# Ham3798/shielded-pool-pinocchio-solana

Measured on AMD Instinct MI355X. Metric: Groth16 proofs/sec, higher is better.
Workload: dtype u32x8 (254-bit Montgomery integers); 1 GPU; audit_circuit (RLWE, const-PK; scripts/generate_audit.py:246-465), batch of 2048 independent proofs per GPU per step, every row a distinct witness; circuit=audit, n_constraints=29178, n_wires=35432, domain=32768, batch_per_gpu=2048, n_distinct_witnesses=2048, table_bytes=226725433344, parallelism=independent proofs x1, pk_bytes=9850060

## Files before the change

### shielded-pool-pinocchio-solana_amd/csrc/bn254.hpp

```cpp
#pragma once
#include <stdint.h>
#include <stddef.h>
#include "bn254_consts.hpp"

#if defined(__HIPCC__)
#include <hip/hip_runtime.h>
#define SPP_HD __host__ __device__ __forceinline__
#define SPP_UNROLL _Pragma("unroll")
#else
#define SPP_HD inline
#define SPP_UNROLL
#endif

namespace spp {

SPP_HD uint32_t addc32(uint32_t a, uint32_t b, uint32_t& carry) {
#if defined(__clang__)
  unsigned co;
  uint32_t r = __builtin_addc(a, b, carry, &co);
  carry = co;
  return r;
#else
  uint64_t t = (uint64_t)a + b + carry;
  carry = (uint32_t)(t >> 32);
// ... 175 lines not shown
    to9(l, a9);
    SPP_UNROLL for (int i = 0; i < 9; i++) d9[i] = a9[i] << 1;
    uint64_t c[18];
    SPP_UNROLL for (int k = 0; k < 18; k++) c[k] = 0;
    SPP_UNROLL for (int i = 0; i < 9; i++) {
      c[2 * i] += (uint64_t)a9[i] * a9[i];
      SPP_UNROLL for (int j = i + 1; j < 9; j++) c[i + j] += (uint64_t)a9[i] * d9[j];
    }
    return reduce_columns(c);
  }

  SPP_HD Fp mul_small(uint32_t k) const {
    Fp acc = zero();
    Fp base = *this;
    while (k) {
      if (k & 1) acc = acc + base;
      base = base.dbl();
      k >>= 1;
    }
    return acc;
  }

  SPP_HD void to_canonical(uint32_t out[8]) const {
    Fp o;
    SPP_UNROLL for (int i = 0; i < 8; i++) o.l[i] = (i == 0);
    Fp c = *this * o;
    cond_sub(c.l);
    SPP_UNROLL for (int i = 0; i < 8; i++) out[i] = c.l[i];
  }
  static SPP_HD Fp from_canonical(const uint32_t in[8]) {
    Fp a;
    SPP_UNROLL for (int i = 0; i < 8; i++) a.l[i] = in[i];
    return a * r2();
  }
  static SPP_HD Fp from_u256(const uint32_t in[8]) {
    Fp a;
    SPP_UNROLL for (int i = 0; i < 8; i++) a.l[i] = in[i];
    for (int k = 0; k < 6; k++) cond_sub(a.l);
    return a * r2();
  }
  static SPP_HD Fp from_u64(uint64_t v) {
    uint32_t c[8];
    SPP_UNROLL for (int i = 0; i < 8; i++) c[i] = 0;
    c[0] = (uint32_t)v;
    c[1] = (uint32_t)(v >> 32);
    return from_canonical(c);
  }
  SPP_HD void to_bytes_be(uint8_t out[32]) const {
    uint32_t c[8];
// ... 339 lines not shown
```

### shielded-pool-pinocchio-solana_amd/csrc/kernels.hpp

```cpp
#pragma once
#include <hip/hip_runtime.h>
#include <stdint.h>
#include "bn254.hpp"
#include "f29.hpp"
#include "msm_plan.hpp"
#include "msm_ragged.hpp"
#include "rlwe_ntt.hpp"

namespace spp {

struct DevSparse {
  const uint32_t* rowptr;
  const uint32_t* wire;
  const uint32_t* coeff;
  const uint32_t* lit;
};
static constexpr uint32_t COEFF_ONE = 0x80000000u;
static constexpr uint32_t COEFF_MINUS_ONE = 0x40000000u;
static constexpr uint32_t COEFF_MASK = 0x3fffffffu;

struct HashConsts {
  const Fr* pos3_rc;  const Fr* pos3_mds;
  const Fr* pos5_rc;  const Fr* pos5_mds;
  const Fr* p2_rc;    const Fr* p2_mu;
  const uint32_t* pos3_mds29;
  const uint32_t* pos5_mds29;
};

struct DevCircuit {
  DevSparse A, B, C, H;
  const Fr* coeffs;
  const Fr* aux;
  const uint32_t* program;
  uint32_t n_wires, n_constraints, n_public, n_inputs, challenge_wire;
  const uint32_t* run_start;
  uint32_t n_runs;
  uint32_t max_row_terms;
  const uint8_t* row_flags;
  const uint32_t* sm_wires;
  const int32_t* sm_lo;
  uint32_t sm_nslots;
  const uint32_t* sm_rowptr;
  const uint32_t* sm_slot;
  const int32_t* sm_coef;
  const uint32_t* sm_rest_ptr;
  const uint32_t* sm_rest_wire;
  const uint32_t* sm_rest_coeff;
  const uint32_t* sm_row_out;
  uint32_t sm_nrows;
  const uint8_t* row_small;
  const uint32_t* lg_rows;
  uint32_t lg_n;
  const uint8_t* row_long;
  HashConsts hc;
// ... 112 lines not shown
void launch_scale_rows(hipStream_t st, Fr* data, const Fr* table, uint32_t n, uint32_t P, uint32_t nbatch, size_t batch_stride);
void launch_qap_pointwise(hipStream_t st, Fr* abc, uint32_t n, uint32_t P, Fr zinv);
void launch_qap_product(hipStream_t st, Fr* abc, uint32_t n, uint32_t P);

template <class F>
struct MsmWalk;
template <>
struct MsmWalk<Fq> {
  static constexpr uint32_t waves_per_simd = 3;
  static constexpr uint32_t rows_waves_per_simd = 2;
  static constexpr int product_form = F29_SCAN;
  static constexpr uint32_t occ(uint32_t Wt) { return Wt == 1 ? waves_per_simd : rows_waves_per_simd; }
};
template <>
struct MsmWalk<Fq2> {
  static constexpr uint32_t waves_per_simd = 2;
  static constexpr uint32_t rows_waves_per_simd = 1;
  static constexpr int product_form = F29_COLUMNS;
  static constexpr uint32_t occ(uint32_t Wt) { return Wt == 1 ? waves_per_simd : rows_waves_per_simd; }
};
template <class F>
void launch_build_table(hipStream_t st, const Affine<F>* bases, uint32_t N, uint32_t c, uint32_t Wt, uint32_t row0, uint32_t nrows,
                        Affine<F>* table, XYZZ<F>* tmp, F* tmp_pre, const MsmBlock* blocks = nullptr, uint32_t E = 0);
void launch_msm_digits(hipStream_t st, const uint32_t* rows, const Fr* scalars, int16_t* dig, uint32_t N, uint32_t P, uint32_t c);
template <class F>
void launch_msm_accumulate(hipStream_t st, const Affine<F>* table, const MsmBlock* blocks, const int16_t* dig, XYZZ<F>* partial, uint32_t N, uint32_t P,
                           uint32_t c, const MsmPlan& pl, hipEvent_t ev_start = nullptr, hipEvent_t ev_stop = nullptr, uint32_t* redo_count = nullptr);
template <class F>
void launch_msm_reduce(hipStream_t st, XYZZ<F>* partial, XYZZ<F>* out, uint32_t P, const MsmPlan& pl, uint32_t c, bool empty);
static constexpr uint32_t MSM_FOLD_SETS = 8;
static constexpr uint32_t MSM_FOLD_RADIX = 8;
template <class F>
struct MsmFoldSets {
  XYZZ<F>* partial[MSM_FOLD_SETS];
  XYZZ<F>* out[MSM_FOLD_SETS];
  uint32_t Sg[MSM_FOLD_SETS], R[MSM_FOLD_SETS], c[MSM_FOLD_SETS];
  uint32_t cur[MSM_FOLD_SETS], half[MSM_FOLD_SETS];
};
template <class F>
void launch_msm_reduce_multi(hipStream_t st, MsmFoldSets<F> fs, uint32_t nsets, uint32_t P);

void launch_g1_eval_basis(hipStream_t st, const G1Affine* pts, uint32_t n_pts, uint32_t logn, const Fr* scale, const Fr* tw_inv, G1XYZZ* work,
                          G1Affine* out);

void launch_g1_column_sums(hipStream_t st, const G1Affine* base, const uint32_t* row, const Fr* coeff, uint32_t nterms, const uint32_t* seg,
                           uint32_t nseg, G1XYZZ* work, G1Affine* out);

// ... 31 lines not shown
```

### shielded-pool-pinocchio-solana_amd/csrc/kernels_msm.hip

```cpp
#include "msm_table.hpp"

namespace spp {

template void launch_build_table<Fq>(hipStream_t, const Affine<Fq>*, uint32_t, uint32_t, uint32_t, uint32_t, uint32_t, Affine<Fq>*,
                                     XYZZ<Fq>*, Fq*, const MsmBlock*, uint32_t);
template void launch_msm_accumulate<Fq>(hipStream_t, const Affine<Fq>*, const MsmBlock*, const int16_t*, XYZZ<Fq>*, uint32_t, uint32_t, uint32_t,
                                        const MsmPlan&, hipEvent_t, hipEvent_t, uint32_t*);
template void launch_msm_reduce_multi<Fq>(hipStream_t, MsmFoldSets<Fq>, uint32_t, uint32_t);
template void launch_msm_reduce<Fq>(hipStream_t, XYZZ<Fq>*, XYZZ<Fq>*, uint32_t, const MsmPlan&, uint32_t, bool);
template void launch_fixed_base_mul<Fq>(hipStream_t, const Affine<Fq>*, uint32_t, const Fr*, uint32_t, Affine<Fq>*);

__global__ void __launch_bounds__(256) k_msm_digits(const uint32_t* __restrict__ rows, const Fr* __restrict__ scalars,
                                                    int16_t* __restrict__ dig, uint32_t N, uint32_t P, uint32_t Pp, uint32_t c, uint32_t W) {
  const uint64_t g = (uint64_t)blockIdx.x * blockDim.x + threadIdx.x;
  const uint32_t p = (uint32_t)(g % Pp), i = (uint32_t)(g / Pp);
  if (i >= N || p >= P) return;
  const Fr s = scalars[(size_t)rows[i] * P + p];
  uint32_t l[8];
  s.to_canonical(l);
  const bool neg = canonical_gt_half<FrParams>(l);
  if (neg) {
    uint32_t t[8];
    canonical_negate<FrParams>(l, t);
    SPP_UNROLL for (int k = 0; k < 8; k++) l[k] = t[k];
  }
  const uint32_t mask = (1u << c) - 1u, half = 1u << (c - 1);
  uint32_t carry = 0;
  int16_t* out = dig + (size_t)i * Pp + p;
  const size_t plane = (size_t)N * Pp;
#pragma unroll 1
  for (uint32_t j = 0; j < W; j++) {
    const uint32_t d = (l[0] & mask) + carry;
    SPP_UNROLL for (int k = 0; k < 7; k++) l[k] = (l[k] >> c) | (l[k + 1] << (32 - c));
    l[7] >>= c;
    const bool over = neg ? d > half : d >= half;
    int v = over ? (int)d - (int)(1u << c) : (int)d;
    carry = over ? 1u : 0u;
    if (neg) v = -v;
    out[(size_t)j * plane] = (int16_t)v;
  }
}
void launch_msm_digits(hipStream_t st, const uint32_t* rows, const Fr* scalars, int16_t* dig, uint32_t N, uint32_t P, uint32_t c) {
  if (N == 0 || P == 0) return;
  const uint32_t Pp = msm_padded_batch(P);
  const uint64_t lanes = (uint64_t)N * Pp;
  hipLaunchKernelGGL(k_msm_digits, dim3((uint32_t)((lanes + 255) / 256)), dim3(256), 0, st, rows, scalars, dig, N, P, Pp, c, msm_windows(c));
}

__device__ __forceinline__ XYZZ<Fq> g1_scalar_mul(const XYZZ<Fq>& pt, const Fr& k) {
  uint32_t c[8];
  k.to_canonical(c);
  XYZZ<Fq> acc = XYZZ<Fq>::infinity();
  if (pt.is_inf()) return acc;
#pragma unroll 1
  for (int w = 7; w >= 0; w--) {
    const uint32_t word = w == 0 ? c[0] : w == 1 ? c[1] : w == 2 ? c[2] : w == 3 ? c[3] : w == 4 ? c[4] : w == 5 ? c[5] : w == 6 ? c[6] : c[7];
#pragma unroll 1
    for (int bit = 31; bit >= 0; bit--) {
      acc.dbl_inplace();
      if ((word >> bit) & 1) acc.add(pt);
    }
  }
  return acc;
}
__global__ void __launch_bounds__(64) k_g1_dft_load(const G1Affine* __restrict__ pts, uint32_t n_pts, const Fr* __restrict__ scale,
                                                    G1XYZZ* __restrict__ x, uint32_t n) {
  const uint32_t j = blockIdx.x * blockDim.x + threadIdx.x;
  if (j >= n) return;
  x[j] = j < n_pts ? g1_scalar_mul(G1XYZZ::from_affine(pts[j]), scale[j]) : G1XYZZ::infinity();
// ... 51 lines not shown
```

### shielded-pool-pinocchio-solana_amd/csrc/kernels_solve.hip

```cpp
#include "kernels.hpp"
#include "circuit.hpp"
#include "poseidon29.hpp"
#include "poseidon2.hpp"
#include "gnark_hints.hpp"
#include "sha256.hpp"

namespace spp {

__device__ __forceinline__ Fr dev_row_dot(const DevSparse& m, const Fr* __restrict__ coeffs, uint32_t k, uint32_t k_end_skip,
                                           const Fr* __restrict__ W, uint32_t P, uint32_t p, uint32_t first = 0, uint32_t step = 1) {
  Fr acc = Fr::zero();
  const uint32_t b = m.rowptr[k] + first, e = m.rowptr[k + 1] - k_end_skip;
  for (uint32_t t = b; t < e; t += step) {
    const uint32_t ci = m.coeff[t];
    Fr w = W[(size_t)m.wire[t] * P + p];
    if (ci & COEFF_ONE) acc = acc + w;
    else if (ci & COEFF_MINUS_ONE) acc = acc - w;
    else acc = acc + coeffs[ci & COEFF_MASK] * w;
  }
  return acc;
}

__global__ void __launch_bounds__(256) k_load_inputs(const uint8_t* __restrict__ in_be, const uint8_t* __restrict__ rs_be,
                                                     Fr* __restrict__ W, uint32_t n_inputs, uint32_t n_wires, uint32_t P) {
// ... 699 lines not shown
  if (lanes) hipLaunchKernelGGL(k_count8_hist, dim3((uint32_t)((lanes + 255) / 256)), dim3(256), 0, st, dc, W, counters, h0, n, P);
  hipLaunchKernelGGL(k_count8_store, dim3((256 * P + 255) / 256), dim3(256), 0, st, counters, W, out0, P);
}

__device__ __forceinline__ void wide_mac(uint32_t (&acc)[10], uint32_t c, const Fr& x) {
  uint32_t carry = 0;
  SPP_UNROLL for (int i = 0; i < 8; i++) {
    const uint64_t t = (uint64_t)c * x.l[i] + acc[i] + carry;
    acc[i] = (uint32_t)t;
    carry = (uint32_t)(t >> 32);
  }
  const uint64_t t = (uint64_t)acc[8] + carry;
  acc[8] = (uint32_t)t;
  acc[9] += (uint32_t)(t >> 32);
}
__device__ __forceinline__ Fr wide_finish(const uint32_t (&acc)[10]) {
  Fr lo;
  SPP_UNROLL for (int i = 0; i < 8; i++) lo.l[i] = acc[i];
  Fr::cond_sub_2p(lo.l);
  Fr::cond_sub_2p(lo.l);
  if ((acc[8] | acc[9]) == 0) return lo;
  return lo + Fr::from_u64((uint64_t)acc[8] | ((uint64_t)acc[9] << 32));
}
__device__ __forceinline__ Fr dev_row_dot_wide(const DevSparse& m, const Fr* __restrict__ coeffs, uint32_t k, const Fr* __restrict__ W,
                                                uint32_t P, uint32_t p, uint32_t first = 0, uint32_t step = 1) {
  Fr acc = Fr::zero();
  uint32_t pos[10], neg[10];
  SPP_UNROLL for (int i = 0; i < 10; i++) pos[i] = neg[i] = 0;
  bool any = false;
  const uint32_t b = m.rowptr[k] + first, e = m.rowptr[k + 1];
  for (uint32_t t = b; t < e; t += step) {
    const uint32_t ci = m.coeff[t], li = m.lit[t];
    const Fr w = W[(size_t)m.wire[t] * P + p];
    if (ci & COEFF_ONE) acc = acc + w;
    else if (ci & COEFF_MINUS_ONE) acc = acc - w;
    else if (li) {
      any = true;
      if (li & 0x80000000u) wide_mac(neg, li & 0x7fffffffu, w);
      else wide_mac(pos, li, w);
    } else acc = acc + coeffs[ci & COEFF_MASK] * w;
  }
  if (any) acc = acc + wide_finish(pos) - wide_finish(neg);
  return acc;
}

__global__ void __launch_bounds__(256) k_small_extract(DevCircuit dc, const Fr* __restrict__ W, int16_t* __restrict__ small, uint32_t P,
                                                       uint32_t* __restrict__ status) {
  const uint64_t g = (uint64_t)blockIdx.x * blockDim.x + threadIdx.x;
  if (g >= (uint64_t)dc.sm_nslots * P) return;
  const uint32_t p = (uint32_t)(g % P), s = (uint32_t)(g / P);
  uint32_t c[8], n[8];
  W[(size_t)dc.sm_wires[s] * P + p].to_canonical(c);
  canonical_negate<FrParams>(c, n);
  const bool pos = (c[1] | c[2] | c[3] | c[4] | c[5] | c[6] | c[7]) == 0 && c[0] < 32768u;
  const bool neg = (n[1] | n[2] | n[3] | n[4] | n[5] | n[6] | n[7]) == 0 && n[0] <= 32768u && (c[0] | c[1] | c[2] | c[3] | c[4] | c[5] | c[6] | c[7]) != 0;
  int v = pos ? (int)c[0] : neg ? -(int)n[0] : 0;
  const int lo = dc.sm_lo[s];
  if ((!pos && !neg) || v < lo || v > lo + 255) {
    atomicOr(&status[p], 1u);
    v = 0;
  }
  small[g] = (int16_t)v;
}
__global__ void __launch_bounds__(256) k_spmv_small_rows(DevCircuit dc, const int16_t* __restrict__ small, const Fr* __restrict__ W,
// ... 7 lines not shown
  const uint32_t ro = dc.sm_row_out[r], mat = ro >> 30, k = ro & 0x3fffffffu;
  const Fr mag = Fr::from_u64((uint64_t)(acc < 0 ? -acc : acc));
  Fr v = acc < 0 ? mag.neg() : mag;
  for (uint32_t t = dc.sm_rest_ptr[r]; t < dc.sm_rest_ptr[r + 1]; t++) v = v + dc.coeffs[dc.sm_rest_coeff[t]] * W[(size_t)dc.sm_rest_wire[t] * P + p];
  abc[(size_t)mat * n * P + (size_t)k * P + p] = v;
}

__global__ void __launch_bounds__(256) k_spmv_check(DevCircuit dc, const Fr* __restrict__ W, Fr* __restrict__ abc, uint32_t n, uint32_t P,
                                                    uint32_t* __restrict__ status) {
  const uint64_t g = (uint64_t)blockIdx.x * blockDim.x + threadIdx.x;
  const uint64_t lanes = (uint64_t)(dc.n_runs + (n - dc.n_constraints)) * P;
  if (g >= lanes) return;
  const uint32_t p = (uint32_t)(g % P), r = (uint32_t)(g / P);
  const uint64_t total = (uint64_t)n * P;
  if (r >= dc.n_runs) {
    const uint64_t o = (uint64_t)(dc.n_constraints + (r - dc.n_runs)) * P + p;
    abc[o] = Fr::zero();
    abc[total + o] = Fr::zero();
    abc[2 * total + o] = Fr::zero();
    return;
  }
  const uint32_t k0 = dc.run_start[r], k1 = dc.run_start[r + 1];
  const uint8_t* __restrict__ rs = dc.row_small;
  const Fr b = (rs && (rs[k0] & 2)) ? abc[total + (uint64_t)k0 * P + p] : dev_row_dot_wide(dc.B, dc.coeffs, k0, W, P, p);
  bool bad = false;
  for (uint32_t k = k0; k < k1; k++) {
    const uint64_t o = (uint64_t)k * P + p;
    const uint32_t f = rs ? rs[k] : 0u;
    const Fr a = (f & 1) ? abc[o] : dev_row_dot_wide(dc.A, dc.coeffs, k, W, P, p);
    const Fr c = (f & 4) ? abc[2 * total + o] : dev_row_dot_wide(dc.C, dc.coeffs, k, W, P, p);
    bad |= (a * b != c);
    abc[o] = a;
    abc[total + o] = b;
    abc[2 * total + o] = c;
  }
  if (bad) atomicOr(&status[p], 1u);
}
static constexpr uint32_t LONG_G = 16;
__global__ void __launch_bounds__(1024) k_spmv_long_rows(DevCircuit dc, const Fr* __restrict__ W, Fr* __restrict__ abc, uint32_t n, uint32_t P) {
  __shared__ Fr part[LONG_G][64];
  const uint32_t lane = threadIdx.x & 63, sub = threadIdx.x >> 6, p = blockIdx.x * 64 + lane;
  const uint32_t code = dc.lg_rows[blockIdx.y], mi = code >> 30, k = code & 0x3fffffffu;
  const DevSparse& m = mi == 0 ? dc.A : mi == 1 ? dc.B : dc.C;
  part[sub][lane] = p < P ? dev_row_dot_wide(m, dc.coeffs, k, W, P, p, sub, LONG_G) : Fr::zero();
  __syncthreads();
  if (sub != 0 || p >= P) return;
  Fr acc = part[0][lane];
  SPP_UNROLL for (uint32_t q = 1; q < LONG_G; q++) acc = acc + part[q][lane];
  abc[(uint64_t)mi * n * P + (uint64_t)k * P + p] = acc;
}

static constexpr uint32_t SPMV_G = 16;
__device__ __forceinline__ Fr group_sum(Fr v) {
  SPP_UNROLL for (uint32_t off = SPMV_G / 2; off >= 1; off >>= 1) {
    Fr o;
    SPP_UNROLL for (int i = 0; i < 8; i++) o.l[i] = __shfl_xor(v.l[i], off);
    v = v + o;
  }
  return v;
}
__global__ void __launch_bounds__(256) k_spmv_check_rows(DevCircuit dc, const Fr* __restrict__ W, Fr* __restrict__ abc, uint32_t n, uint32_t P,
                                                         uint32_t* __restrict__ status) {
  const uint64_t g = (uint64_t)blockIdx.x * blockDim.x + threadIdx.x;
  const uint64_t total = (uint64_t)n * P;
  const uint64_t e = g / SPMV_G;
  const uint32_t sub = (uint32_t)(g % SPMV_G);
  const bool live = e < total;
  const uint32_t p = live ? (uint32_t)(e % P) : 0, k = live ? (uint32_t)(e / P) : dc.n_constraints;
  Fr a = Fr::zero(), b = Fr::zero(), c = Fr::zero();
  if (k < dc.n_constraints) {
    a = dev_row_dot_wide(dc.A, dc.coeffs, k, W, P, p, sub, SPMV_G);
    b = dev_row_dot_wide(dc.B, dc.coeffs, k, W, P, p, sub, SPMV_G);
    c = dev_row_dot_wide(dc.C, dc.coeffs, k, W, P, p, sub, SPMV_G);
  }
  a = group_sum(a);
  b = group_sum(b);
  c = group_sum(c);
  if (!live || sub != 0) return;
  if (a * b != c) atomicOr(&status[p], 1u);
  abc[e] = a;
  abc[total + e] = b;
  abc[2 * total + e] = c;
}
void launch_spmv_check(hipStream_t st, DevCircuit dc, const Fr* W, Fr* abc, uint32_t n, uint32_t P, uint32_t* status, int16_t* small) {
  if ((uint64_t)dc.n_runs * P < 65536 || (P <= 64 && dc.max_row_terms > 1024)) {
    const uint64_t lanes = (uint64_t)n * P * SPMV_G;
    hipLaunchKernelGGL(k_spmv_check_rows, dim3((uint32_t)((lanes + 255) / 256)), dim3(256), 0, st, dc, W, abc, n, P, status);
    return;
  }
  if (small && dc.sm_nrows) {
    const uint64_t l1 = (uint64_t)dc.sm_nslots * P, l2 = (uint64_t)dc.sm_nrows * P;
    hipLaunchKernelGGL(k_small_extract, dim3((uint32_t)((l1 + 255) / 256)), dim3(256), 0, st, dc, W, small, P, status);
    hipLaunchKernelGGL(k_spmv_small_rows, dim3((uint32_t)((l2 + 255) / 256)), dim3(256), 0, st, dc, small, W, abc, n, P);
  } else {
    dc.row_small = dc.row_long;
  }
// ... 7 lines not shown
```

### shielded-pool-pinocchio-solana_amd/csrc/msm_table.hpp

```cpp
#pragma once
#include <hip/hip_ext.h>
#include "kernels.hpp"
#include <algorithm>
#include "f29.hpp"

namespace spp {

static constexpr unsigned MSM_FOLD_COOP_MAX_BATCH = 8;
static constexpr unsigned MSM_WALK_BLOCK = 64;

template <class F>
__global__ void __launch_bounds__(64) k_build_table(const Affine<F>* __restrict__ bases, uint32_t N, uint32_t E, uint32_t Wn,
                                                    uint32_t step_bits, uint32_t row0, uint32_t nrows, Affine<F>* __restrict__ table,
                                                    XYZZ<F>* __restrict__ tmp, F* __restrict__ tmp_pre, const MsmBlock* __restrict__ blocks) {
  const uint32_t rl = blockIdx.x * blockDim.x + threadIdx.x;
  if (rl >= nrows) return;
  const uint32_t row = row0 + rl;
  const size_t off = blocks ? (size_t)blocks[row >> 6].off : (size_t)(row >> 6) * E;
  Affine<F>* out = table + off * 64 + (row & 63);
  XYZZ<F>* t = tmp + rl;
  F* pre = tmp_pre + rl;
  if (row >= N * Wn) {
    for (uint32_t d = 0; d < E; d++) out[(size_t)d * 64] = Affine<F>::infinity();
    return;
  }
  const uint32_t i = row / Wn, j = row % Wn;
  Affine<F> base = bases[i];
// ... 404 lines not shown
```

### shielded-pool-pinocchio-solana_amd/csrc/spp_load.cpp

```cpp
#include "spp_circuit.hpp"

static std::vector<PendingTable<Fq>>& pending(spp_circuit* c, Fq*) { return c->pending1; }
static std::vector<PendingTable<Fq2>>& pending(spp_circuit* c, Fq2*) { return c->pending2; }

static int upload_sparse(spp_circuit* c, const Circuit& circ, const Sparse& m, DevSparse* out) {
  std::vector<uint32_t> wire(m.terms.size()), coeff(m.terms.size()), lit(m.terms.size(), 0);
  Fr one = Fr::one(), mone = Fr::one().neg();
  std::vector<uint32_t> small(circ.coeffs.size(), 0);
  for (size_t ci = 0; ci < circ.coeffs.size(); ci++) {
    uint32_t v[8], nv[8];
    circ.coeffs[ci].to_canonical(v);
    bool hi0 = true;
    for (int k = 1; k < 8; k++) hi0 = hi0 && v[k] == 0;
    if (hi0 && v[0] != 0 && v[0] < (1u << 28)) { small[ci] = v[0]; continue; }
    circ.coeffs[ci].neg().to_canonical(nv);
    hi0 = true;
    for (int k = 1; k < 8; k++) hi0 = hi0 && nv[k] == 0;
    if (hi0 && nv[0] != 0 && nv[0] < (1u << 28)) small[ci] = nv[0] | 0x80000000u;
  }
  for (size_t i = 0; i < m.terms.size(); i++) {
    wire[i] = m.terms[i].wire;
    uint32_t ci = m.terms[i].coeff;
    uint32_t flag = 0;
    if (circ.coeffs[ci] == one) flag = COEFF_ONE;
// ... 256 lines not shown
      sets.push_back(plan_set(s, nset[s], flat[s]));
    }
    const std::vector<uint32_t>* keyed[7] = {&pk.A_w, &pk.B1_w, &pk.K_w, nullptr, nullptr, nullptr, &pk.B2_w};
    for (int s = 0; s < 7; s++)
      if (keyed[s] && flat[s])
        for (uint32_t b : msm_base_bounds(wc, *keyed[s])) plan_count(sets[s], b);
    plan_greedy(sets, budget, use_flat ? 16 : 15);
    for (int s = 0; s < 7; s++) cw[s] = (uint32_t)sets[s].bits;
  }
  return 0;
}

static int load_r1cs(spp_circuit* c) {
  const Circuit& circ = c->circ;
  int e;
  if ((e = upload_sparse(c, circ, circ.A, &c->dc.A)) || (e = upload_sparse(c, circ, circ.B, &c->dc.B)) ||
      (e = upload_sparse(c, circ, circ.C, &c->dc.C)) || (e = upload_sparse(c, circ, circ.H, &c->dc.H)))
    return e;
  Fr* d_coeffs;
  Fr* d_aux;
  uint32_t* d_prog;
  if ((e = own_upload(c, &d_coeffs, circ.coeffs)) || (e = own_upload(c, &d_prog, circ.program)) || (e = own_upload(c, &d_aux, circ.aux))) return e;
  c->dc.coeffs = d_coeffs;
  c->dc.aux = d_aux;
  c->dc.program = d_prog;
  c->dc.n_wires = circ.n_wires;
  c->dc.n_constraints = circ.n_constraints;
  {
    std::vector<uint32_t> runs;
    auto same_b = [&](uint32_t k) {
      const uint32_t a0 = circ.B.rowptr[k - 1], a1 = circ.B.rowptr[k], b1 = circ.B.rowptr[k + 1];
      if (a1 - a0 != b1 - a1 || a1 == a0) return false;
      for (uint32_t t = 0; t < a1 - a0; t++)
        if (circ.B.terms[a0 + t].wire != circ.B.terms[a1 + t].wire || circ.B.terms[a0 + t].coeff != circ.B.terms[a1 + t].coeff) return false;
      return true;
    };
    uint32_t len = 0;
    for (uint32_t k = 0; k < circ.n_constraints; k++) {
      if (k == 0 || len >= 8 || !same_b(k)) { runs.push_back(k); len = 0; }
      len++;
    }
    const uint32_t n_runs = (uint32_t)runs.size();
    runs.push_back(circ.n_constraints);
    uint32_t* d_runs;
    if ((e = own_upload(c, &d_runs, runs))) return e;
    c->dc.run_start = d_runs;
// ... 526 lines not shown
  }
  std::vector<MsmBlock> blocks(msm_table_rows(n, 1) / 64);
  for (size_t b = 0; b < blocks.size(); b++) blocks[b] = {(uint64_t)b * E, E, 0};
  spp_circuit tmpc;
  tmpc.ctx = ctx;
  tmpc.c_bits = cb;
  Affine<F>* table = nullptr;
  int e = build_table_chunked<F>(&tmpc, pts, cb, 1, &table);
  Fr* d_sc = nullptr;
  uint32_t* d_rows = nullptr;
  MsmBlock* d_blocks = nullptr;
  const MsmPlan pl = msm_plan(N, Pn, cb, 1, MsmWalk<F>::occ(1), read_switches().msm);
  DevBuf partial, d_out, dig, count;
  if (!e) e = own_upload(&tmpc, &d_sc, sc);
  if (!e) e = own_upload(&tmpc, &d_rows, rows);
  if (!e) e = own_upload(&tmpc, &d_blocks, blocks);
  if (!e && (partial.alloc(sizeof(XYZZ<F>) * pl.partial_elems(Pn)) != hipSuccess || d_out.alloc(sizeof(XYZZ<F>) * P) != hipSuccess ||
             dig.alloc(sizeof(int16_t) * msm_digit_elems(N, Pn, cb)) != hipSuccess || count.alloc(sizeof(uint32_t)) != hipSuccess))
    e = fail(SPP_ERR_HIP, "hipMalloc");
  std::vector<XYZZ<F>> res(P);
  uint32_t redone = 0;
  if (!e) {
    hipMemsetAsync(count.p, 0, sizeof(uint32_t), st);
    launch_msm_digits(st, d_rows, d_sc, dig.as<int16_t>(), N, Pn, cb);
    launch_msm_accumulate<F>(st, table, d_blocks, dig.as<int16_t>(), partial.as<XYZZ<F>>(), N, Pn, cb, pl, nullptr, nullptr, count.as<uint32_t>());
    launch_msm_reduce<F>(st, partial.as<XYZZ<F>>(), d_out.as<XYZZ<F>>(), Pn, pl, cb, false);
    if (hipStreamSynchronize(st) != hipSuccess || hipGetLastError() != hipSuccess) e = fail(SPP_ERR_HIP, "msm kernels failed");
    else if (hipMemcpy(res.data(), d_out.p, sizeof(XYZZ<F>) * P, hipMemcpyDeviceToHost) != hipSuccess ||
             hipMemcpy(&redone, count.p, sizeof redone, hipMemcpyDeviceToHost) != hipSuccess)
      e = fail(SPP_ERR_HIP, "copy back failed");
  }
  for (void* p : tmpc.owned) hipFree(p);
  if (e) return e;
  for (size_t p = 0; p < P; p++) point_to_raw(res[p].to_affine(), out + PT_BYTES * p);
  if (redo_lanes) *redo_lanes = redone;
  return SPP_OK;
}
extern "C" int spp_msm_flat_unit(spp_ctx* ctx, int group, const uint8_t* bases, size_t n, const uint8_t* scalars, size_t P, int window_bits,
                                 uint8_t* out, uint32_t* redo_lanes) {
  if (group == 1) return msm_flat_unit<Fq, 64>(ctx, bases, n, scalars, P, window_bits, out, redo_lanes);
  if (group == 2) return msm_flat_unit<Fq2, 128>(ctx, bases, n, scalars, P, window_bits, out, redo_lanes);
  return fail(SPP_ERR_BAD_INPUT, "group is 1 or 2");
}
```

### shielded-pool-pinocchio-solana_amd/csrc/spp_prove.cpp

```cpp
#include "spp_circuit.hpp"

template <class T>
static int ws_alloc(Workspace& w, T** p, size_t count) {
  HIP_TRY(hipMalloc((void**)p, sizeof(T) * std::max<size_t>(count, 1)));
  w.owned.push_back((void*)*p);
  return 0;
}
template <class F>
static int ws_set(const spp_circuit* c, Workspace& w, const MsmSet<F>* s, MsmBuf<F>* b, size_t P) {
  b->partial_cap = msm_partial_cap(s->N, P, s->c, s->Wt, MsmWalk<F>::occ(s->Wt), c->sw.msm);
  int e;
  if ((e = ws_alloc(w, &b->partial, b->partial_cap))) return e;
  return ws_alloc(w, &b->out, P);
}
static int ensure_workspace(spp_circuit* c, Workspace& w, size_t P) {
  if (P <= w.cap) return 0;
  HIP_TRY(hipStreamSynchronize(w.st));
  free_workspace(w);
  int e;
  if ((e = ws_alloc(w, &w.W, (size_t)c->n_rows * P)) || (e = ws_alloc(w, &w.abc, (size_t)3 * c->n * P)) ||
      (e = ws_alloc(w, &w.scratch, (size_t)c->max_batch_div * P)) || (e = ws_alloc(w, &w.commit_affine, P)) ||
      (e = ws_alloc(w, &w.d_inputs, c->in_stride * P)) || (e = ws_alloc(w, &w.d_rs, 64 * P)) ||
      (e = ws_alloc(w, &w.d_proofs, (size_t)SPP_PROOF_LEN * P)) || (e = ws_alloc(w, &w.d_pws, c->pw_stride * P)) ||
      (e = ws_alloc(w, &w.d_status, P)) || (e = ws_alloc(w, &w.counters, 256 * P)))
// ... 14 lines not shown
    w.dig1_cap = d1;
    w.dig2_cap = msm_digit_elems(c->B2.N, (uint32_t)P, c->B2.c);
    if ((e = ws_alloc(w, &w.dig1, w.dig1_cap)) || (e = ws_alloc(w, &w.dig2, w.dig2_cap))) return e;
    if (c->dc.sm_nrows && (e = ws_alloc(w, &w.small, (size_t)c->dc.sm_nslots * P))) return e;
  }
  w.cap = P;
  return 0;
}

static int16_t* ws_dig(Workspace& w, Fq*) { return w.dig1; }
static int16_t* ws_dig(Workspace& w, Fq2*) { return w.dig2; }
template <class F>
static void run_msm(spp_circuit* c, Workspace& w, const MsmSet<F>& s, MsmBuf<F>& b, uint32_t P, bool timed, hipStream_t st_override = nullptr,
                    std::pair<hipEvent_t, hipEvent_t>* ev_override = nullptr, bool fold = true, const Fr* scal_override = nullptr) {
  hipStream_t st = st_override ? st_override : w.st;
  const Fr* scal = scal_override ? scal_override : s.from_h ? w.abc : w.W;
  MsmPlan pl = msm_plan(s.N, P, s.c, s.Wt, MsmWalk<F>::occ(s.Wt), c->sw.msm);
  pl.fit(P, b.partial_cap);
  b.plan = pl;
  std::pair<hipEvent_t, hipEvent_t>* ev = nullptr;
  if (timed && w.msm_ev_used < w.msm_ev.size()) ev = &w.msm_ev[w.msm_ev_used++];
  if (ev_override) ev = ev_override;
  int16_t* dig = ws_dig(w, (F*)nullptr);
  launch_msm_digits(st, s.rows, scal, dig, s.N, P, s.c);
  launch_msm_accumulate<F>(st, s.table, s.blocks, dig, b.partial, s.N, P, s.c, pl, ev ? ev->first : nullptr, ev ? ev->second : nullptr);
  if (fold) launch_msm_reduce<F>(st, b.partial, b.out, P, pl, s.c, s.N == 0);
}

static int prove_on_device(spp_circuit* c, Workspace& w, uint32_t P, const uint8_t* d_inputs, const uint8_t* d_rs, uint8_t* d_proofs,
                           uint8_t* d_pws, uint32_t* d_status) {
  hipStream_t st = w.st;
  const Circuit& circ = c->circ;
  const uint32_t n = c->n;
  w.msm_ev_used = 0;
  w.last_P = P;
  const bool scaled_blind = P <= scaled_blind_max_batch(c->A.N, c->B1.N) && !c->sw.no_coop && !c->A.narrow && !c->B1.narrow;
  HIP_TRY(hipMemsetAsync(d_status, 0, sizeof(uint32_t) * P, st));
  hipEventRecord(w.ev[0], st);
  launch_load_inputs(st, d_inputs, d_rs, w.W, circ.n_inputs(), circ.n_wires, P);
  hipEventRecord(w.ev_in, st);
  for (const SolveStep& s : c->schedule) {
    switch (s.kind) {
      case SolveStep::SEQ:
        if (P <= c->sw.coop_max_batch && !c->sw.no_coop && c->sw.trace_items) {
          for (uint32_t t = 0; t < s.ntracks; t++)
            for (uint32_t it = s.tr_begin[t]; it < s.tr_end[t]; it++) {
              CoopTracks one{};
// ... 480 lines not shown
```

Baseline: 7494 proofs/s.

## Speed up Fr-side work: cheaper canonical conversion, lazy row dot products, narrow digit recoding

to_canonical now runs Montgomery reduction directly on the limbs and no longer multiplies by one. Sparse row dot products with general coefficients now gather 29-bit limb columns with a precomputed coeffs29 table and do one lazy reduction per chunk, not a full Fp multiply per term. The MSM digit kernel gets an unrolled c=16 path and a narrow-block shortcut that writes a single digit and zeros when the block's bound fits in one window. It also adds profiling scripts. The risks are correctness of the scaled-by-32 coefficient representation and of the narrow shortcut, plus extra coefficient table memory.

After: 7587 proofs/s, median of 6. 1.01x the previous value.

```diff
diff --git a/profiles/fr_side_accounting.py b/profiles/fr_side_accounting.py
--- /dev/null
+++ b/profiles/fr_side_accounting.py
@@ -0,0 +1,43 @@
+#!/usr/bin/env python3
+import re
+import sys
+
+from f29_scan_accounting import kernels, loop_blocks
+
+KERNELS = ("k_msm_digits", "k_spmv_check_rows", "k_spmv_long_rows", "k_spmv_check", "k_ntt_pass")
+
+
+def pretty(sym):
+    for name in KERNELS:
+        if "%d%s" % (len(name), name) in sym:
+            if name == "k_ntt_pass":
+                return name + ("<DIF>" if "ILb1E" in sym else "<DIT>")
+            return name
+    return None
+
+
+def lds_bytes(path, sym):
+    m = re.search(r"\.amdhsa_kernel %s\b.*?\.amdhsa_group_segment_fixed_size (\d+)" % re.escape(sym), open(path).read(), re.S)
+    return int(m.group(1)) if m else None
+
+
+def main():
+    print("%-8s %-20s %6s %6s %6s %6s %6s %6s %6s %5s %5s %8s %6s %5s" % ("commit", "kernel", "instr", "inloop", "mad64", "add64", "shr64", "mul32",
+                                                                         "global", "lds", "VGPR", "scratch", "LDS_B", "waves"))
+    for arg in sys.argv[1:]:
+        label, path = arg.split(":", 1)
+        for sym, (body, res) in sorted(kernels(open(path).read()).items()):
+            name = pretty(sym)
+            if not name:
+                continue
+            ops = [op for b in loop_blocks(body + ["s_branch .LBB_all"], whole=True) for op in b]
+            inloop = sum(len(b) for b in loop_blocks(body))
+            add = ops.count("v_lshl_add_u64") + sum(1 for op in ops if op.startswith("v_addc_co_u32"))
+            print("%-8s %-20s %6d %6d %6d %6d %6d %6d %6d %5d %5s %8s %6s %5s" % (
+                label, name, len(ops), inloop, ops.count("v_mad_u64_u32"), add, ops.count("v_lshrrev_b64"), ops.count("v_mul_lo_u32"),
+                sum(1 for op in ops if op.startswith("global_")), sum(1 for op in ops if op.startswith("ds_")), res.get("vgpr"),
+                res.get("scratch"), lds_bytes(path, sym), res.get("occ")))
+
+
+if __name__ == "__main__":
+    main()
diff --git a/profiles/fr_side_term_kinds.cpp b/profiles/fr_side_term_kinds.cpp
--- /dev/null
+++ b/profiles/fr_side_term_kinds.cpp
@@ -0,0 +1,123 @@
+#include <cstdio>
+#include <cstdlib>
+#include <vector>
+#include "circuit.hpp"
+#include "msm_classes.hpp"
+using namespace spp;
+
+static void count_matrix(const char* circ_name, const char* name, const Circuit& c, const Sparse& m) {
+  const Fr one = Fr::one(), mone = Fr::one().neg();
+  std::vector<uint8_t> kind(c.coeffs.size(), 2);
+  for (size_t ci = 0; ci < c.coeffs.size(); ci++) {
+    int64_t v;
+    if (c.coeffs[ci] == one || c.coeffs[ci] == mone) kind[ci] = 0;
+    else if (fr_small_signed(c.coeffs[ci], &v) && v != 0 && (v < 0 ? -v : v) < (1 << 28)) kind[ci] = 1;
+  }
+  size_t n[3] = {0, 0, 0}, rows_general = 0, hist[5] = {0, 0, 0, 0, 0}, max_general = 0;
+  for (uint32_t r = 0; r < m.rows(); r++) {
+    size_t g = 0;
+    for (uint32_t t = m.rowptr[r]; t < m.rowptr[r + 1]; t++) {
+      n[kind[m.terms[t].coeff]]++;
+      g += kind[m.terms[t].coeff] == 2;
+    }
+    if (g) rows_general++;
+    hist[g == 0 ? 0 : g == 1 ? 1 : g == 2 ? 2 : g <= 6 ? 3 : 4]++;
+    if (g > max_general) max_general = g;
+  }
+  printf("%-9s %s  rows %6u  terms %7zu  +-1 %7zu  small literal %7zu  general %7zu | rows with general terms %6zu (1: %zu, 2: %zu, 3-6: %zu, 7+: %zu, most %zu)\n",
+         circ_name, name, m.rows(), m.terms.size(), n[0], n[1], n[2], rows_general, hist[1], hist[2], hist[3], hist[4], max_general);
+}
+static void count_small_rows(const char* name, const Circuit& c);
+static void count_sets(const char* name, const Circuit& c);
+static void count_circuit(const char* name, const Circuit& c) {
+  count_matrix(name, "A", c, c.A);
+  count_matrix(name, "B", c, c.B);
+  count_matrix(name, "C", c, c.C);
+  const WireClasses wc = msm_wire_classes(c);
+  size_t k[4] = {0, 0, 0, 0};
+  for (uint32_t w = 0; w < c.n_wires; w++) k[wc.kind[w]]++;
+  printf("%-9s wires %u: wide %zu, bits %zu, bytes (limbs) %zu, looked-up bytes %zu -> narrow %.1f %%\n", name, c.n_wires, k[WIRE_WIDE], k[WIRE_BIT],
+         k[WIRE_LIMB8], k[WIRE_LOOKUP], 100.0 * (double)(k[1] + k[2] + k[3]) / (double)c.n_wires);
+  count_small_rows(name, c);
+  count_sets(name, c);
+}
+
+static void count_small_rows(const char* name, const Circuit& c) {
+  std::vector<uint8_t> ranged(c.n_wires, 0);
+  ranged[0] = 1;
+  const std::vector<uint32_t>& pr = c.program;
+  for (size_t pc = 0; pc < pr.size() && pr[pc] != OP_END;) {
+    size_t len = 0;
+    switch (pr[pc]) {
+      case OP_SOLVE_C: case OP_SOLVE_A: case OP_MASK: len = 2; break;
+      case OP_BATCH_DIV: case OP_POSEIDON2: case OP_INV_H: len = 3; break;
+      case OP_COUNT8: case OP_BITS: case OP_LIMBS8: case OP_POSEIDON: len = 4; break;
+      case OP_COMMIT: len = 1; break;
+      case OP_GRUMPKIN: len = pc + 4 < pr.size() ? 5 + (size_t)pr[pc + 4] : 0; break;
+      default: len = 0;
+    }
+    if (len == 0 || pc + len > pr.size()) break;
+    if (pr[pc] == OP_COUNT8)
+      for (uint32_t i = 0; i < pr[pc + 2]; i++) {
+        uint32_t w;
+        int64_t cst;
+        if (circuit_byte_ranged_lookup(c, pr[pc + 1] + i, &w, &cst) && w < c.n_wires) ranged[w] = 1;
+      }
+    pc += len;
+  }
+  const Sparse* mats[3] = {&c.A, &c.B, &c.C};
+  const char* mn[3] = {"A", "B", "C"};
+  for (int mi = 0; mi < 3; mi++) {
+    const Sparse& m = *mats[mi];
+    size_t rows = 0, small_terms = 0, rest_terms = 0;
+    for (uint32_t k = 0; k < c.n_constraints && k < m.rows(); k++) {
+      const uint32_t b = m.rowptr[k], e = m.rowptr[k + 1];
+      if (e - b < 64) continue;
+      uint32_t ns = 0;
+      for (uint32_t t = b; t < e; t++) {
+        int64_t v;
+        if (ranged[m.terms[t].wire] && fr_small_signed(c.coeffs[m.terms[t].coeff], &v)) ns++;
+      }
+      if (ns < 64 || (e - b) - ns > 32) continue;
+      rows++;
+      small_terms += ns;
+      rest_terms += (e - b) - ns;
+    }
+    printf("%-9s %s  rows on the small-row path %5zu: %7zu terms summed as integers, %5zu other terms (Fp products in k_spmv_small_rows)\n", name, mn[mi], rows,
+           small_terms, rest_terms);
+  }
+}
+static void count_sets(const char* name, const Circuit& c) {
+  const WireClasses wc = msm_wire_classes(c);
+  std::vector<uint8_t> inA(c.n_wires, 0), inB(c.n_wires, 0), com(c.n_wires, 0);
+  for (const Term& t : c.A.terms) inA[t.wire] = 1;
+  for (const Term& t : c.B.terms) inB[t.wire] = 1;
+  for (uint32_t w : c.committed) if (w < c.n_wires) com[w] = 1;
+  const char* kn[4] = {"wide", "bits", "bytes (limbs)", "looked-up bytes"};
+  for (int set = 0; set < 4; set++) {
+    size_t k[4] = {0, 0, 0, 0}, n = 0;
+    for (uint32_t w = 0; w < c.n_wires; w++) {
+      const bool in = set == 0 ? inA[w] : set == 1 ? inB[w] : set == 2 ? (w >= c.n_public && !com[w]) : com[w];
+      if (!in) continue;
+      n++;
+      k[wc.kind[w]]++;
+    }
+    printf("%-9s set %-7s %6zu wires:", name, set == 0 ? "A" : set == 1 ? "B1, B2" : set == 2 ? "K" : "CB, CS", n);
+    for (int q = 0; q < 4; q++) printf(" %s %zu,", kn[q], k[q]);
+    printf(" narrow %.1f %%\n", n ? 100.0 * (double)(k[1] + k[2] + k[3]) / (double)n : 0.0);
+  }
+}
+
+int main(int argc, char** argv) {
+  count_circuit("withdraw", build_withdraw_circuit(true));
+  if (argc > 1) {
+    std::vector<uint32_t> pk;
+    FILE* f = fopen(argv[1], "r");
+    unsigned v;
+    while (f && fscanf(f, "%u", &v) == 1) pk.push_back(v);
+    if (f) fclose(f);
+    if (pk.size() != 2048) { fprintf(stderr, "need 2048 pk coefficients\n"); return 2; }
+    count_circuit("audit", build_audit_circuit(pk.data(), pk.data() + 1024, true));
+  }
+  return 0;
+}
diff --git a/shielded-pool-pinocchio-solana_amd/csrc/bn254.hpp b/shielded-pool-pinocchio-solana_amd/csrc/bn254.hpp
--- a/shielded-pool-pinocchio-solana_amd/csrc/bn254.hpp
+++ b/shielded-pool-pinocchio-solana_amd/csrc/bn254.hpp
@@ -221,9 +221,11 @@
   }
 
   SPP_HD void to_canonical(uint32_t out[8]) const {
-    Fp o;
-    SPP_UNROLL for (int i = 0; i < 8; i++) o.l[i] = (i == 0);
-    Fp c = *this * o;
+    uint32_t a9[9];
+    to9(l, a9);
+    uint64_t col[18];
+    SPP_UNROLL for (int k = 0; k < 18; k++) col[k] = k < 9 ? a9[k] : 0;
+    Fp c = reduce_columns(col);
     cond_sub(c.l);
     SPP_UNROLL for (int i = 0; i < 8; i++) out[i] = c.l[i];
   }
diff --git a/shielded-pool-pinocchio-solana_amd/csrc/kernels.hpp b/shielded-pool-pinocchio-solana_amd/csrc/kernels.hpp
--- a/shielded-pool-pinocchio-solana_amd/csrc/kernels.hpp
+++ b/shielded-pool-pinocchio-solana_amd/csrc/kernels.hpp
@@ -3,6 +3,7 @@
 #include <stdint.h>
 #include "bn254.hpp"
 #include "f29.hpp"
+#include "row_cols.hpp"
 #include "msm_plan.hpp"
 #include "msm_ragged.hpp"
 #include "rlwe_ntt.hpp"
@@ -30,6 +31,7 @@
 struct DevCircuit {
   DevSparse A, B, C, H;
   const Fr* coeffs;
+  const uint32_t* coeffs29;
   const Fr* aux;
   const uint32_t* program;
   uint32_t n_wires, n_constraints, n_public, n_inputs, challenge_wire;
@@ -188,7 +190,8 @@
 template <class F>
 void launch_build_table(hipStream_t st, const Affine<F>* bases, uint32_t N, uint32_t c, uint32_t Wt, uint32_t row0, uint32_t nrows,
                         Affine<F>* table, XYZZ<F>* tmp, F* tmp_pre, const MsmBlock* blocks = nullptr, uint32_t E = 0);
-void launch_msm_digits(hipStream_t st, const uint32_t* rows, const Fr* scalars, int16_t* dig, uint32_t N, uint32_t P, uint32_t c);
+void launch_msm_digits(hipStream_t st, const uint32_t* rows, const Fr* scalars, int16_t* dig, uint32_t N, uint32_t P, uint32_t c,
+                       const MsmBlock* blocks = nullptr);
 template <class F>
 void launch_msm_accumulate(hipStream_t st, const Affine<F>* table, const MsmBlock* blocks, const int16_t* dig, XYZZ<F>* partial, uint32_t N, uint32_t P,
                            uint32_t c, const MsmPlan& pl, hipEvent_t ev_start = nullptr, hipEvent_t ev_stop = nullptr, uint32_t* redo_count = nullptr);
diff --git a/shielded-pool-pinocchio-solana_amd/csrc/kernels_msm.hip b/shielded-pool-pinocchio-solana_amd/csrc/kernels_msm.hip
--- a/shielded-pool-pinocchio-solana_amd/csrc/kernels_msm.hip
+++ b/shielded-pool-pinocchio-solana_amd/csrc/kernels_msm.hip
@@ -11,40 +11,25 @@
 template void launch_fixed_base_mul<Fq>(hipStream_t, const Affine<Fq>*, uint32_t, const Fr*, uint32_t, Affine<Fq>*);
 
 __global__ void __launch_bounds__(256) k_msm_digits(const uint32_t* __restrict__ rows, const Fr* __restrict__ scalars,
-                                                    int16_t* __restrict__ dig, uint32_t N, uint32_t P, uint32_t Pp, uint32_t c, uint32_t W) {
+                                                    int16_t* __restrict__ dig, const MsmBlock* __restrict__ blocks, uint32_t N, uint32_t P,
+                                                    uint32_t Pp, uint32_t c, uint32_t W) {
   const uint64_t g = (uint64_t)blockIdx.x * blockDim.x + threadIdx.x;
   const uint32_t p = (uint32_t)(g % Pp), i = (uint32_t)(g / Pp);
   if (i >= N || p >= P) return;
-  const Fr s = scalars[(size_t)rows[i] * P + p];
-  uint32_t l[8];
-  s.to_canonical(l);
-  const bool neg = canonical_gt_half<FrParams>(l);
-  if (neg) {
-    uint32_t t[8];
-    canonical_negate<FrParams>(l, t);
-    SPP_UNROLL for (int k = 0; k < 8; k++) l[k] = t[k];
-  }
-  const uint32_t mask = (1u << c) - 1u, half = 1u << (c - 1);
-  uint32_t carry = 0;
+  const bool narrow = blocks && blocks[i >> 6].E < (1u << (c - 1));
   int16_t* out = dig + (size_t)i * Pp + p;
   const size_t plane = (size_t)N * Pp;
-#pragma unroll 1
-  for (uint32_t j = 0; j < W; j++) {
-    const uint32_t d = (l[0] & mask) + carry;
-    SPP_UNROLL for (int k = 0; k < 7; k++) l[k] = (l[k] >> c) | (l[k + 1] << (32 - c));
-    l[7] >>= c;
-    const bool over = neg ? d > half : d >= half;
-    int v = over ? (int)d - (int)(1u << c) : (int)d;
-    carry = over ? 1u : 0u;
-    if (neg) v = -v;
-    out[(size_t)j * plane] = (int16_t)v;
-  }
+  msm_scalar_digits(scalars[(size_t)rows[i] * P + p], c, W, narrow, [&](uint32_t, int16_t v) {
+    *out = v;
+    out += plane;
+  });
 }
-void launch_msm_digits(hipStream_t st, const uint32_t* rows, const Fr* scalars, int16_t* dig, uint32_t N, uint32_t P, uint32_t c) {
+void launch_msm_digits(hipStream_t st, const uint32_t* rows, const Fr* scalars, int16_t* dig, uint32_t N, uint32_t P, uint32_t c,
+                       const MsmBlock* blocks) {
   if (N == 0 || P == 0) return;
   const uint32_t Pp = msm_padded_batch(P);
   const uint64_t lanes = (uint64_t)N * Pp;
-  hipLaunchKernelGGL(k_msm_digits, dim3((uint32_t)((lanes + 255) / 256)), dim3(256), 0, st, rows, scalars, dig, N, P, Pp, c, msm_windows(c));
+  hipLaunchKernelGGL(k_msm_digits, dim3((uint32_t)((lanes + 255) / 256)), dim3(256), 0, st, rows, scalars, dig, blocks, N, P, Pp, c, msm_windows(c));
 }
 
 __device__ __forceinline__ XYZZ<Fq> g1_scalar_mul(const XYZZ<Fq>& pt, const Fr& k) {
diff --git a/shielded-pool-pinocchio-solana_amd/csrc/kernels_solve.hip b/shielded-pool-pinocchio-solana_amd/csrc/kernels_solve.hip
--- a/shielded-pool-pinocchio-solana_amd/csrc/kernels_solve.hip
+++ b/shielded-pool-pinocchio-solana_amd/csrc/kernels_solve.hip
@@ -745,12 +745,14 @@
   if ((acc[8] | acc[9]) == 0) return lo;
   return lo + Fr::from_u64((uint64_t)acc[8] | ((uint64_t)acc[9] << 32));
 }
-__device__ __forceinline__ Fr dev_row_dot_wide(const DevSparse& m, const Fr* __restrict__ coeffs, uint32_t k, const Fr* __restrict__ W,
+__device__ __forceinline__ Fr dev_row_dot_wide(const DevSparse& m, const uint32_t* __restrict__ coeffs29, uint32_t k, const Fr* __restrict__ W,
                                                 uint32_t P, uint32_t p, uint32_t first = 0, uint32_t step = 1) {
   Fr acc = Fr::zero();
   uint32_t pos[10], neg[10];
   SPP_UNROLL for (int i = 0; i < 10; i++) pos[i] = neg[i] = 0;
   bool any = false;
+  RowCols cols;
+  cols.init();
   const uint32_t b = m.rowptr[k] + first, e = m.rowptr[k + 1];
   for (uint32_t t = b; t < e; t += step) {
     const uint32_t ci = m.coeff[t], li = m.lit[t];
@@ -761,8 +763,9 @@
       any = true;
       if (li & 0x80000000u) wide_mac(neg, li & 0x7fffffffu, w);
       else wide_mac(pos, li, w);
-    } else acc = acc + coeffs[ci & COEFF_MASK] * w;
-  }
+    } else cols.term(w, coeffs29 + (size_t)(ci & COEFF_MASK) * 9, acc);
+  }
+  cols.flush(acc);
   if (any) acc = acc + wide_finish(pos) - wide_finish(neg);
   return acc;
 }
@@ -816,13 +819,13 @@
   }
   const uint32_t k0 = dc.run_start[r], k1 = dc.run_start[r + 1];
   const uint8_t* __restrict__ rs = dc.row_small;
-  const Fr b = (rs && (rs[k0] & 2)) ? abc[total + (uint64_t)k0 * P + p] : dev_row_dot_wide(dc.B, dc.coeffs, k0, W, P, p);
+  const Fr b = (rs && (rs[k0] & 2)) ? abc[total + (uint64_t)k0 * P + p] : dev_row_dot_wide(dc.B, dc.coeffs29, k0, W, P, p);
   bool bad = false;
   for (uint32_t k = k0; k < k1; k++) {
     const uint64_t o = (uint64_t)k * P + p;
     const uint32_t f = rs ? rs[k] : 0u;
-    const Fr a = (f & 1) ? abc[o] : dev_row_dot_wide(dc.A, dc.coeffs, k, W, P, p);
-    const Fr c = (f & 4) ? abc[2 * total + o] : dev_row_dot_wide(dc.C, dc.coeffs, k, W, P, p);
+    const Fr a = (f & 1) ? abc[o] : dev_row_dot_wide(dc.A, dc.coeffs29, k, W, P, p);
+    const Fr c = (f & 4) ? abc[2 * total + o] : dev_row_dot_wide(dc.C, dc.coeffs29, k, W, P, p);
     bad |= (a * b != c);
     abc[o] = a;
     abc[total + o] = b;
@@ -836,7 +839,7 @@
   const uint32_t lane = threadIdx.x & 63, sub = threadIdx.x >> 6, p = blockIdx.x * 64 + lane;
   const uint32_t code = dc.lg_rows[blockIdx.y], mi = code >> 30, k = code & 0x3fffffffu;
   const DevSparse& m = mi == 0 ? dc.A : mi == 1 ? dc.B : dc.C;
-  part[sub][lane] = p < P ? dev_row_dot_wide(m, dc.coeffs, k, W, P, p, sub, LONG_G) : Fr::zero();
+  part[sub][lane] = p < P ? dev_row_dot_wide(m, dc.coeffs29, k, W, P, p, sub, LONG_G) : Fr::zero();
   __syncthreads();
   if (sub != 0 || p >= P) return;
   Fr acc = part[0][lane];
@@ -863,9 +866,9 @@
   const uint32_t p = live ? (uint32_t)(e % P) : 0, k = live ? (uint32_t)(e / P) : dc.n_constraints;
   Fr a = Fr::zero(), b = Fr::zero(), c = Fr::zero();
   if (k < dc.n_constraints) {
-    a = dev_row_dot_wide(dc.A, dc.coeffs, k, W, P, p, sub, SPMV_G);
-    b = dev_row_dot_wide(dc.B, dc.coeffs, k, W, P, p, sub, SPMV_G);
-    c = dev_row_dot_wide(dc.C, dc.coeffs, k, W, P, p, sub, SPMV_G);
+    a = dev_row_dot_wide(dc.A, dc.coeffs29, k, W, P, p, sub, SPMV_G);
+    b = dev_row_dot_wide(dc.B, dc.coeffs29, k, W, P, p, sub, SPMV_G);
+    c = dev_row_dot_wide(dc.C, dc.coeffs29, k, W, P, p, sub, SPMV_G);
   }
   a = group_sum(a);
   b = group_sum(b);
diff --git a/shielded-pool-pinocchio-solana_amd/csrc/msm_recode.hpp b/shielded-pool-pinocchio-solana_amd/csrc/msm_recode.hpp
--- /dev/null
+++ b/shielded-pool-pinocchio-solana_amd/csrc/msm_recode.hpp
@@ -0,0 +1,59 @@
+#pragma once
+#include "bn254.hpp"
+
+namespace spp {
+
+SPP_HD int msm_signed_digit(uint32_t d, bool neg, uint32_t c, uint32_t& carry) {
+  const uint32_t half = 1u << (c - 1);
+  const bool over = neg ? d > half : d >= half;
+  const int v = over ? (int)d - (int)(1u << c) : (int)d;
+  carry = over ? 1u : 0u;
+  return neg ? -v : v;
+}
+template <class Store>
+SPP_HD void msm_recode_digits(const uint32_t (&mag)[8], bool neg, uint32_t c, uint32_t W, Store&& store) {
+  uint32_t carry = 0;
+  if (c == 16 && W == 16) {
+    SPP_UNROLL for (uint32_t j = 0; j < 16; j++) {
+      const uint32_t d = ((mag[j >> 1] >> (16 * (j & 1))) & 0xffffu) + carry;
+      store(j, (int16_t)msm_signed_digit(d, neg, 16, carry));
+    }
+    return;
+  }
+  uint32_t l[8];
+  SPP_UNROLL for (int k = 0; k < 8; k++) l[k] = mag[k];
+  const uint32_t mask = (1u << c) - 1u;
+#if defined(__HIP_DEVICE_COMPILE__)
+#pragma unroll 1
+#endif
+  for (uint32_t j = 0; j < W; j++) {
+    const uint32_t d = (l[0] & mask) + carry;
+    SPP_UNROLL for (int k = 0; k < 7; k++) l[k] = (l[k] >> c) | (l[k + 1] << (32 - c));
+    l[7] >>= c;
+    store(j, (int16_t)msm_signed_digit(d, neg, c, carry));
+  }
+}
+
+template <class Store>
+SPP_HD void msm_scalar_digits(const Fr& s, uint32_t c, uint32_t W, bool narrow, Store&& store) {
+  uint32_t l[8], mag[8];
+  s.to_canonical(l);
+  const bool neg = canonical_gt_half<FrParams>(l);
+  if (neg) {
+    canonical_negate<FrParams>(l, mag);
+  } else {
+    SPP_UNROLL for (int k = 0; k < 8; k++) mag[k] = l[k];
+  }
+  if (narrow) {
+    uint32_t carry = 0;
+    store(0u, (int16_t)msm_signed_digit(mag[0] & ((1u << c) - 1u), neg, c, carry));
+#if defined(__HIP_DEVICE_COMPILE__)
+#pragma unroll 1
+#endif
+    for (uint32_t j = 1; j < W; j++) store(j, (int16_t)0);
+    return;
+  }
+  msm_recode_digits(mag, neg, c, W, store);
+}
+
+}
diff --git a/shielded-pool-pinocchio-solana_amd/csrc/msm_table.hpp b/shielded-pool-pinocchio-solana_amd/csrc/msm_table.hpp
--- a/shielded-pool-pinocchio-solana_amd/csrc/msm_table.hpp
+++ b/shielded-pool-pinocchio-solana_amd/csrc/msm_table.hpp
@@ -3,6 +3,7 @@
 #include "kernels.hpp"
 #include <algorithm>
 #include "f29.hpp"
+#include "msm_recode.hpp"
 
 namespace spp {
 
diff --git a/shielded-pool-pinocchio-solana_amd/csrc/row_cols.hpp b/shielded-pool-pinocchio-solana_amd/csrc/row_cols.hpp
--- /dev/null
+++ b/shielded-pool-pinocchio-solana_amd/csrc/row_cols.hpp
@@ -0,0 +1,49 @@
+#pragma once
+#include "f29.hpp"
+
+namespace spp {
+
+static constexpr uint32_t ROW_COLS_CHUNK = 7;
+static constexpr uint32_t ROW_COLS_FLUSH = 126;
+
+SPP_HD void row_coeff29(const Fr& c, uint32_t out[9]) {
+  const Fr s = (c * Fr::from_u64(32)).canonical();
+  Fr::to9(s.l, out);
+}
+
+struct RowCols {
+  using F = F29<FrParams>;
+  uint64_t c[18];
+  uint32_t n;
+  SPP_HD void init() {
+    F::clear(c);
+    n = 0;
+  }
+  SPP_HD void term(const Fr& w, const uint32_t* coeff29, Fr& acc) {
+    F k;
+    SPP_UNROLL for (int i = 0; i < 9; i++) k.l[i] = coeff29[i];
+    F::mac(c, F::from_words(w.l), k);
+    n++;
+    if (n % ROW_COLS_CHUNK == 0) {
+      if (n == ROW_COLS_FLUSH) flush(acc);
+      else fold();
+    }
+  }
+  SPP_HD void fold() {
+    SPP_UNROLL for (int k = 0; k < 17; k++) {
+      c[k + 1] += c[k] >> 29;
+      c[k] &= F::M;
+    }
+  }
+  SPP_HD void flush(Fr& acc) {
+    if (n == 0) return;
+    const F r = F::reduce(c);
+    Fr o;
+    r.to_words(o.l);
+    Fr::cond_sub_2p(o.l);
+    acc = acc + o;
+    init();
+  }
+};
+
+}
diff --git a/shielded-pool-pinocchio-solana_amd/csrc/spp_load.cpp b/shielded-pool-pinocchio-solana_amd/csrc/spp_load.cpp
--- a/shielded-pool-pinocchio-solana_amd/csrc/spp_load.cpp
+++ b/shielded-pool-pinocchio-solana_amd/csrc/spp_load.cpp
@@ -302,6 +302,13 @@
   uint32_t* d_prog;
   if ((e = own_upload(c, &d_coeffs, circ.coeffs)) || (e = own_upload(c, &d_prog, circ.program)) || (e = own_upload(c, &d_aux, circ.aux))) return e;
   c->dc.coeffs = d_coeffs;
+  {
+    std::vector<uint32_t> c29(circ.coeffs.size() * 9);
+    for (size_t ci = 0; ci < circ.coeffs.size(); ci++) row_coeff29(circ.coeffs[ci], &c29[ci * 9]);
+    uint32_t* d_c29;
+    if ((e = own_upload(c, &d_c29, c29))) return e;
+    c->dc.coeffs29 = d_c29;
+  }
   c->dc.aux = d_aux;
   c->dc.program = d_prog;
   c->dc.n_wires = circ.n_wires;
@@ -874,7 +881,7 @@
   uint32_t redone = 0;
   if (!e) {
     hipMemsetAsync(count.p, 0, sizeof(uint32_t), st);
-    launch_msm_digits(st, d_rows, d_sc, dig.as<int16_t>(), N, Pn, cb);
+    launch_msm_digits(st, d_rows, d_sc, dig.as<int16_t>(), N, Pn, cb, d_blocks);
     launch_msm_accumulate<F>(st, table, d_blocks, dig.as<int16_t>(), partial.as<XYZZ<F>>(), N, Pn, cb, pl, nullptr, nullptr, count.as<uint32_t>());
     launch_msm_reduce<F>(st, partial.as<XYZZ<F>>(), d_out.as<XYZZ<F>>(), Pn, pl, cb, false);
     if (hipStreamSynchronize(st) != hipSuccess || hipGetLastError() != hipSuccess) e = fail(SPP_ERR_HIP, "msm kernels failed");
diff --git a/shielded-pool-pinocchio-solana_amd/csrc/spp_prove.cpp b/shielded-pool-pinocchio-solana_amd/csrc/spp_prove.cpp
--- a/shielded-pool-pinocchio-solana_amd/csrc/spp_prove.cpp
+++ b/shielded-pool-pinocchio-solana_amd/csrc/spp_prove.cpp
@@ -60,7 +60,7 @@
   if (timed && w.msm_ev_used < w.msm_ev.size()) ev = &w.msm_ev[w.msm_ev_used++];
   if (ev_override) ev = ev_override;
   int16_t* dig = ws_dig(w, (F*)nullptr);
-  launch_msm_digits(st, s.rows, scal, dig, s.N, P, s.c);
+  launch_msm_digits(st, s.rows, scal, dig, s.N, P, s.c, s.blocks);
   launch_msm_accumulate<F>(st, s.table, s.blocks, dig, b.partial, s.N, P, s.c, pl, ev ? ev->first : nullptr, ev ? ev->second : nullptr);
   if (fold) launch_msm_reduce<F>(st, b.partial, b.out, P, pl, s.c, s.N == 0);
 }
```
